# manyeyes/K2TransducerAsr

Measured on AMD Instinct MI355X. Metric: RTFx (audio-sec/wall-sec) offline Zipformer greedy, higher is better.
Workload: dtype f32

## Files before the change

### k2transducerasr_amd/csrc/elementwise.hip

```cpp
#include "kernels.h"

namespace k2hip {
namespace {

constexpr float kLogFloor = -23.025850929940457F;

__device__ __forceinline__ float fast_softplus(float z) { return z > 15.f ? z : __logf(1.0f + __expf(z)); }
__device__ __forceinline__ float swoosh_r(float v) { return fast_softplus(v - 1.0f) - 0.08f * v - 0.313261687f; }
__device__ __forceinline__ float fast_tanh(float v) {
    float e = __expf(-2.0f * fabsf(v));
    float t = (1.0f - e) / (1.0f + e);
    return v < 0.f ? -t : t;
}

__device__ __forceinline__ float sigm(float s) { return 1.0f / (1.0f + __expf(-s)); }
__device__ __forceinline__ float dswish(float v) { return v / (1.0f + __expf(1.0f - v)); }

inline int nblocks(long long n, int per) { return (int)((n + per - 1) / per); }

__global__ void k_pad_logfloor(const float* __restrict__ packed, const long long* __restrict__ off,
                               const long long* __restrict__ len, float* __restrict__ out, long long L) {
    int b = blockIdx.y;
    const float* src = packed + off[b];
    long long n = len[b];
    for (long long j = (long long)blockIdx.x * blockDim.x + threadIdx.x; j < L; j += (long long)gridDim.x * blockDim.x) {
        float v = j < n ? src[j] : 0.0f;
        out[(long long)b * L + j] = (v == 0.0f) ? kLogFloor : v;
    }
}
__global__ void k_pad_logfloor_dense(const float* __restrict__ feats, long long n, float* __restrict__ out, long long L) {
    int b = blockIdx.y;
    for (long long j = (long long)blockIdx.x * blockDim.x + threadIdx.x; j < L; j += (long long)gridDim.x * blockDim.x) {
        float v = j < n ? feats[(long long)b * n + j] : 0.0f;
        out[(long long)b * L + j] = (v == 0.0f) ? kLogFloor : v;
    }
}

template <int TPAD, bool DSWISH>
__global__ void k_conv0(const float* __restrict__ x, const float* __restrict__ w, const float* __restrict__ bias,
                        float* __restrict__ y, int B, int T, int F) {
    __shared__ float sw[72], sb[8];
    if (threadIdx.x < 72) sw[threadIdx.x] = w[threadIdx.x];
    if (threadIdx.x < 8) sb[threadIdx.x] = bias[threadIdx.x];
    __syncthreads();
    int T1 = T - 2 + 2 * TPAD;
    long long n = (long long)B * T1 * F;
    long long i = (long long)blockIdx.x * blockDim.x + threadIdx.x;
    if (i >= n) return;
    int f = (int)(i % F);
    long long bt = i / F;
    int t = (int)(bt % T1), b = (int)(bt / T1);
    float xin[3][3];
#pragma unroll
    for (int kt = 0; kt < 3; kt++)
#pragma unroll
        for (int kf = 0; kf < 3; kf++) {
            int ff = f + kf - 1, tt = t + kt - TPAD;
            xin[kt][kf] = (ff >= 0 && ff < F && tt >= 0 && tt < T) ? x[((long long)b * T + tt) * F + ff] : 0.f;
// ... 719 lines not shown
```

### k2transducerasr_amd/csrc/engine.cpp

```cpp
#include <cstring>
#include <thread>

#include "engine.h"

#include <climits>
#include <cmath>

namespace k2hip {

namespace {
constexpr int kTailFrames = 19;
}

Engine::Engine(const std::string& weights, const char* overrides, int device) : device_(device) {
    tunables_init_from_env();
    model_.reset(new Model(weights, overrides));
    int n = 0;
    if (hipGetDeviceCount(&n) != hipSuccess || n <= 0)
        failf(K2HIP_ERR_NO_DEVICE, "no HIP device visible: libk2hip has no CPU fallback");
    if (device < 0 || device >= n) failf(K2HIP_ERR_NO_DEVICE, "device %d out of range (have %d)", device, n);
    K2_HIP(hipSetDevice(device));
    model_->upload(device);
    K2_HIP(hipStreamCreateWithFlags(&stream_, hipStreamNonBlocking));
    K2_HIP(hipStreamCreateWithFlags(&stream2_, hipStreamNonBlocking));
// ... 1065 lines not shown
    run_sized([&](const Ctx& c) {
        Arena& ar = *c.arena;
        d_tok = ar.take<long long>((int64_t)B * max_tokens);
        d_ts = ar.take<int>((int64_t)B * max_tokens);
        d_n = ar.take<int>(B);
        d_ovf = ar.take<int>(1);
        float* d_packed = ar.take<float>(total);
        long long* d_off = ar.take<long long>(B);
        long long* d_len = ar.take<long long>(B);
        float* d_x = ar.take<float>((int64_t)B * L);
        if (!c.dry) {
            K2_HIP(hipEventRecord(ev_[0], c.stream));
            K2_HIP(hipMemcpyAsync(d_packed, pin, sizeof(float) * total, hipMemcpyHostToDevice, c.stream));
            K2_HIP(hipMemcpyAsync(d_off, off.data(), sizeof(long long) * B, hipMemcpyHostToDevice, c.stream));
            K2_HIP(hipMemcpyAsync(d_len, len.data(), sizeof(long long) * B, hipMemcpyHostToDevice, c.stream));
            K2_HIP(hipEventRecord(ev_[1], c.stream));
        }
        pad_logfloor(c, d_packed, d_off, d_len, d_x, B, L);
        if (!c.dry) K2_HIP(hipEventRecord(ev_[2], c.stream));
        int Tp = 0;
        float* enc = encoder_forward(c, d_x, B, T, &Tp, -1, nullptr, nullptr, nullptr);
        if (!c.dry) K2_HIP(hipEventRecord(ev_[3], c.stream));
        greedy_device(c, enc, B, Tp, single, d_tok, d_ts, d_n, max_tokens, d_ovf);
        if (!c.dry) K2_HIP(hipEventRecord(ev_[4], c.stream));
    });
    finish_tokens(d_tok, d_ts, d_n, d_ovf, B, max_tokens, tokens, ts, n_tokens);
    auto el = [&](int a, int b) { float ms = 0; (void)hipEventElapsedTime(&ms, ev_[a], ev_[b]); return ms; };
    timing_.fbank_ms = 0;
    timing_.pad_ms = el(1, 2);
    timing_.encoder_ms = el(2, 3);
    timing_.greedy_ms = el(3, 4);
    timing_.d2h_ms = el(4, 5);
    timing_.total_ms = el(0, 5);
}

void Engine::offline_greedy_samples_dev(const float* samples_dev, int64_t n_each, int B, int64_t* tokens, int32_t* ts,
                                        int32_t* n_tokens, int max_tokens) {
    K2_REQUIRE(B > 0 && max_tokens > 0 && samples_dev != nullptr, "offline_greedy_from_samples: bad arguments");
    const Config& cf = model_->cfg();
    const FbankOpts& f = cf.fbank;
    K2_REQUIRE(cf.ctc || cf.J == 512, "offline loops hard-code a 512-wide encoder_out; joiner_dim is %d", cf.J);
    const int64_t nf = fbank_num_frames(n_each);
    K2_REQUIRE(nf > 0, "offline_greedy_from_samples: %lld samples give no frame", (long long)n_each);
    const int64_t n_fl = nf * cf.feat, L = n_fl + 80 * kTailFrames;
    const int T = (int)(L / cf.feat);
    long long* d_tok = nullptr;
    int *d_ts = nullptr, *d_n = nullptr, *d_ovf = nullptr;
    run_sized([&](const Ctx& c) {
        Arena& ar = *c.arena;
        d_tok = ar.take<long long>((int64_t)B * max_tokens);
        d_ts = ar.take<int>((int64_t)B * max_tokens);
        d_n = ar.take<int>(B);
        d_ovf = ar.take<int>(1);
        float* d_feats = ar.take<float>((int64_t)B * n_fl);
        float* d_x = ar.take<float>((int64_t)B * L);
        if (!c.dry) K2_HIP(hipEventRecord(ev_[0], c.stream));
        FbankArgs a{samples_dev, n_each, n_each, B, nf, d_feats, model_->d_window, model_->d_melw, f.frame_len, f.frame_shift,
                    f.preemph, f.input_scale, f.remove_dc};
        a.melrange = model_->d_melrange;
        fbank(c, a);
        if (!c.dry) K2_HIP(hipEventRecord(ev_[1], c.stream));
        pad_logfloor_dense(c, d_feats, n_fl, d_x, B, L);
        if (!c.dry) K2_HIP(hipEventRecord(ev_[2], c.stream));
        int Tp = 0;
        float* enc = encoder_forward(c, d_x, B, T, &Tp, -1, nullptr, nullptr, nullptr);
        if (!c.dry) K2_HIP(hipEventRecord(ev_[3], c.stream));
        greedy_device(c, enc, B, Tp, false, d_tok, d_ts, d_n, max_tokens, d_ovf);
        if (!c.dry) K2_HIP(hipEventRecord(ev_[4], c.stream));
    });
    finish_tokens(d_tok, d_ts, d_n, d_ovf, B, max_tokens, tokens, ts, n_tokens);
    auto el = [&](int a, int b) { float ms = 0; (void)hipEventElapsedTime(&ms, ev_[a], ev_[b]); return ms; };
    timing_.fbank_ms = el(0, 1);
    timing_.pad_ms = el(1, 2);
    timing_.encoder_ms = el(2, 3);
    timing_.greedy_ms = el(3, 4);
    timing_.d2h_ms = el(4, 5);
    timing_.total_ms = el(0, 5);
}

void Engine::offline_greedy_samples(const float* const* samples, const int64_t* n_samples, int B, int64_t* tokens, int32_t* ts,
                                    int32_t* n_tokens, int max_tokens, bool single, bool pinned_src) {
    K2_REQUIRE(B > 0 && max_tokens > 0, "offline_greedy_from_samples: bad B=%d / max_tokens=%d", B, max_tokens);
    K2_REQUIRE(!single || B == 1, "offline_greedy_from_samples: the single-stream loop takes one stream");
    K2_HIP(hipSetDevice(device_));
    const Config& cf = model_->cfg();
    const FbankOpts& f = cf.fbank;
    K2_REQUIRE(cf.ctc || cf.J == 512, "offline loops hard-code a 512-wide encoder_out (OfflineRecognizer.cs:103,201); joiner_dim is %d", cf.J);
    int64_t nmax = 0;
    for (int b = 0; b < B; b++) {
        K2_REQUIRE(samples[b] != nullptr && fbank_num_frames(n_samples[b]) > 0, "stream %d: %lld samples give no frame", b, (long long)n_samples[b]);
        nmax = std::max(nmax, n_samples[b]);
    }
    const int64_t nfmax = fbank_num_frames(nmax), n_fl = nfmax * cf.feat, L = n_fl + 80 * kTailFrames;
    const int T = (int)(L / cf.feat);
    const int64_t ns = (nmax + 3) & ~(int64_t)3;
    const int64_t nb_s = align_up((int64_t)sizeof(float) * B * ns, 16);
    const int64_t hb_s = pinned_src ? 0 : nb_s, hb_in = hb_s + 32 * (int64_t)B;
    char* pin = static_cast<char*>(pinned(std::max<int64_t>(hb_in, (int64_t)B * max_tokens * 12 + 4 * (int64_t)B + 64) + 64));
    long long* h_off = reinterpret_cast<long long*>(pin + hb_s);
    long long* h_len = h_off + B;
    const float** h_ptr = reinterpret_cast<const float**>(h_len + B);
    long long* h_cnt = reinterpret_cast<long long*>(h_ptr + B);
    if (pinned_src) {
        for (int b = 0; b < B; b++) {
            void* dp = nullptr;
            K2_HIP(hipHostGetDevicePointer(&dp, const_cast<float*>(samples[b]), 0));
            h_ptr[b] = static_cast<const float*>(dp);
            h_cnt[b] = n_samples[b];
        }
    } else {
        auto stage = [&](int b_lo, int b_hi) {
            for (int b = b_lo; b < b_hi; b++) {
                float* row = reinterpret_cast<float*>(pin) + (size_t)b * ns;
                memcpy(row, samples[b], sizeof(float) * (size_t)n_samples[b]);
                if (n_samples[b] < ns) memset(row + n_samples[b], 0, sizeof(float) * (size_t)(ns - n_samples[b]));
            }
        };
        const int64_t stage_bytes = (int64_t)sizeof(float) * B * ns;
        const int helpers = stage_bytes >= (4 << 20) ? std::min(3, B - 1) : 0;
        if (helpers > 0) {
            std::vector<std::thread> th;
            const int per = (B + helpers) / (helpers + 1);
            for (int h = 1; h <= helpers; h++) th.emplace_back(stage, std::min(B, h * per), std::min(B, (h + 1) * per));
            stage(0, std::min(B, per));
            for (auto& t : th) t.join();
        } else {
            stage(0, B);
        }
    }
    for (int b = 0; b < B; b++) {
        h_off[b] = (long long)b * n_fl;
        h_len[b] = fbank_num_frames(n_samples[b]) * cf.feat;
    }
    long long* d_tok = nullptr;
    int *d_ts = nullptr, *d_n = nullptr, *d_ovf = nullptr;
    run_sized([&](const Ctx& c) {
        Arena& ar = *c.arena;
        d_tok = ar.take<long long>((int64_t)B * max_tokens);
        d_ts = ar.take<int>((int64_t)B * max_tokens);
        d_n = ar.take<int>(B);
        d_ovf = ar.take<int>(1);
        char* d_in = ar.take<char>(nb_s + 32 * (int64_t)B);
        float* d_s = reinterpret_cast<float*>(d_in);
        long long* d_off = reinterpret_cast<long long*>(d_in + nb_s);
        long long* d_len = d_off + B;
        const float* const* d_ptr = reinterpret_cast<const float* const*>(d_len + B);
        const long long* d_cnt = reinterpret_cast<const long long*>(d_ptr + B);
        float* d_feats = ar.take<float>((int64_t)B * n_fl);
        float* d_x = ar.take<float>((int64_t)B * L);
        if (!c.dry) {
            K2_HIP(hipEventRecord(ev_[0], c.stream));
            if (pinned_src) K2_HIP(hipMemcpyAsync(d_in + nb_s, pin, (size_t)(32 * (int64_t)B), hipMemcpyHostToDevice, c.stream));
            else K2_HIP(hipMemcpyAsync(d_in, pin, (size_t)(nb_s + 16 * (int64_t)B), hipMemcpyHostToDevice, c.stream));
        }
        if (pinned_src) gather_samples(c, d_ptr, d_cnt, d_s, B, ns);
        FbankArgs a{d_s, nmax, ns, B, nfmax, d_feats, model_->d_window, model_->d_melw, f.frame_len, f.frame_shift,
                    f.preemph, f.input_scale, f.remove_dc};
        a.melrange = model_->d_melrange;
        fbank(c, a);
        if (!c.dry) K2_HIP(hipEventRecord(ev_[1], c.stream));
        pad_logfloor(c, d_feats, d_off, d_len, d_x, B, L);
        if (!c.dry) K2_HIP(hipEventRecord(ev_[2], c.stream));
        int Tp = 0;
        float* enc = encoder_forward(c, d_x, B, T, &Tp, -1, nullptr, nullptr, nullptr);
        if (!c.dry) K2_HIP(hipEventRecord(ev_[3], c.stream));
        greedy_device(c, enc, B, Tp, single, d_tok, d_ts, d_n, max_tokens, d_ovf);
        if (!c.dry) K2_HIP(hipEventRecord(ev_[4], c.stream));
    });
    finish_tokens(d_tok, d_ts, d_n, d_ovf, B, max_tokens, tokens, ts, n_tokens);
    auto el = [&](int a, int b) { float ms = 0; (void)hipEventElapsedTime(&ms, ev_[a], ev_[b]); return ms; };
    timing_.fbank_ms = el(0, 1);
    timing_.pad_ms = el(1, 2);
    timing_.encoder_ms = el(2, 3);
    timing_.greedy_ms = el(3, 4);
    timing_.d2h_ms = el(4, 5);
    timing_.total_ms = el(0, 5);
}

int Engine::submit_samples_dev(const float* samples_dev, int64_t n_each, int B, int max_tokens) {
    K2_REQUIRE(samples_dev != nullptr, "offline_submit: bad arguments");
    return submit_impl(samples_dev, nullptr, n_each, B, max_tokens);
}
int Engine::submit_samples_host(const float* samples_host, int64_t n_each, int B, int max_tokens) {
    K2_REQUIRE(samples_host != nullptr, "offline_submit: bad arguments");
    return submit_impl(nullptr, samples_host, n_each, B, max_tokens);
}

int Engine::submit_impl(const float* samples_dev, const float* samples_host, int64_t n_each, int B, int max_tokens) {
    K2_REQUIRE(B > 0 && max_tokens > 0, "offline_submit: bad arguments");
    const Config& cf = model_->cfg();
    const FbankOpts& f = cf.fbank;
    K2_REQUIRE(cf.ctc || cf.J == 512, "offline loops hard-code a 512-wide encoder_out; joiner_dim is %d", cf.J);
    const int64_t nf = fbank_num_frames(n_each);
    K2_REQUIRE(nf > 0, "offline_submit: %lld samples give no frame", (long long)n_each);
    const bool deep = beam_ > 0 && !cf.ctc;
    const int nslots = deep ? kSlots : 2;
    int ticket = -1, in_flight = 0;
    for (const auto& x : slots_) in_flight += x.busy;
    for (int k = 0; k < kSlots && ticket < 0; k++) {
        const int cand = (next_slot_ + k) % kSlots;
        if (!slots_[cand].busy && cand < nslots) ticket = cand;
    }
    if (ticket < 0 || in_flight >= nslots)
        failf(K2HIP_ERR_INVALID, "offline_submit: %d batches already in flight; wait for one first", in_flight);
    Slot& sl = slots_[ticket];
    if (!sl.stream) K2_HIP(hipStreamCreateWithFlags(&sl.stream, hipStreamNonBlocking));
    const int64_t n_fl = nf * cf.feat, L = n_fl + 80 * kTailFrames;
    const int T = (int)(L / cf.feat);
    const int64_t nb = (int64_t)B * max_tokens * 12 + (int64_t)B * 4 + 64;
    if (nb > sl.pin_cap) {
        if (sl.pin) K2_HIP(hipHostFree(sl.pin));
        sl.pin = nullptr;
        sl.pin_cap = 0;
        K2_HIP(hipHostMalloc(&sl.pin, (size_t)nb, hipHostMallocDefault));
        sl.pin_cap = nb;
    }
    cur_arena_ = &sl.arena;
    hipStream_t s2 = deep ? sl.stream : stream2_;
    try {
        run_sized([&](const Ctx& c) {
            Arena& ar = *c.arena;
            sl.d_tok = ar.take<long long>((int64_t)B * max_tokens);
            sl.d_ts = ar.take<int>((int64_t)B * max_tokens);
            sl.d_n = ar.take<int>(B);
            sl.d_ovf = ar.take<int>(1);
            float* d_feats = ar.take<float>((int64_t)B * n_fl);
            float* d_x = ar.take<float>((int64_t)B * L);
            const float* src = samples_dev;
            if (samples_host) {
                float* d_s = ar.take<float>((int64_t)B * n_each);
                src = d_s;
                if (!c.dry) {
                    hipStream_t cs = deep ? stream2_ : sl.stream;
                    K2_HIP(hipMemcpyAsync(d_s, samples_host, sizeof(float) * (size_t)B * n_each, hipMemcpyHostToDevice, cs));
                    K2_HIP(hipEventRecord(sl.h2d_done, cs));
                    K2_HIP(hipStreamWaitEvent(c.stream, sl.h2d_done, 0));
                }
            }
            FbankArgs a{src, n_each, n_each, B, nf, d_feats, model_->d_window, model_->d_melw, f.frame_len, f.frame_shift,
                        f.preemph, f.input_scale, f.remove_dc};
            a.melrange = model_->d_melrange;
            fbank(c, a);
            pad_logfloor_dense(c, d_feats, n_fl, d_x, B, L);
            int Tp = 0;
            float* enc = encoder_forward(c, d_x, B, T, &Tp, -1, nullptr, nullptr, nullptr);
            Ctx cd = c;
            cd.stream = s2;
            cd.instrument = false;
            cd.greedy_rec = &sl.greedy;
            sl.greedy.valid = false;
            if (!c.dry) {
                K2_HIP(hipEventRecord(sl.enc_done, c.stream));
                K2_HIP(hipStreamWaitEvent(s2, sl.enc_done, 0));
            }
            greedy_device(cd, enc, B, Tp, false, sl.d_tok, sl.d_ts, sl.d_n, max_tokens, sl.d_ovf);
        });
    } catch (...) {
        cur_arena_ = &arena_;
        throw;
    }
    cur_arena_ = &arena_;
    const int64_t nb_tok = (int64_t)B * max_tokens * 8, nb_ts = (int64_t)B * max_tokens * 4, nb_n = (int64_t)B * 4;
    char* pin = static_cast<char*>(sl.pin);
    K2_HIP(hipMemcpyAsync(pin, sl.d_tok, nb_tok, hipMemcpyDeviceToHost, s2));
    K2_HIP(hipMemcpyAsync(pin + nb_tok, sl.d_ts, nb_ts, hipMemcpyDeviceToHost, s2));
    K2_HIP(hipMemcpyAsync(pin + nb_tok + nb_ts, sl.d_n, nb_n, hipMemcpyDeviceToHost, s2));
    K2_HIP(hipMemcpyAsync(pin + nb_tok + nb_ts + nb_n, sl.d_ovf, 4, hipMemcpyDeviceToHost, s2));
    K2_HIP(hipEventRecord(sl.done, s2));
    sl.B = B;
    sl.max_tokens = max_tokens;
    sl.search_stream = s2;
    sl.busy = true;
    next_slot_ = (ticket + 1) % nslots;
    return ticket;
}

void Engine::wait_ticket(int ticket, int64_t* tokens, int32_t* ts, int32_t* n_tokens) {
    K2_REQUIRE(ticket >= 0 && ticket < kSlots && slots_[ticket].busy, "offline_wait: ticket %d is not in flight", ticket);
    K2_HIP(hipSetDevice(device_));
    Slot& sl = slots_[ticket];
    K2_HIP(hipEventSynchronize(sl.done));
    sl.busy = false;
    const int64_t nb_tok = (int64_t)sl.B * sl.max_tokens * 8, nb_ts = (int64_t)sl.B * sl.max_tokens * 4, nb_n = (int64_t)sl.B * 4;
    char* pin = static_cast<char*>(sl.pin);
    int ovf = *reinterpret_cast<const int*>(pin + nb_tok + nb_ts + nb_n);
    note_search(sl.greedy.valid && sl.greedy.a.overflow == sl.d_ovf, ovf == 2 && sl.greedy.valid && sl.greedy.a.overflow == sl.d_ovf);
    if (ovf == 2 && sl.greedy.valid && sl.greedy.a.overflow == sl.d_ovf) {
        hipStream_t s2 = sl.search_stream;
        greedy_relaunch_one_part(s2, sl.greedy);
        search_retries_++;
        K2_HIP(hipMemcpyAsync(pin, sl.d_tok, nb_tok, hipMemcpyDeviceToHost, s2));
        K2_HIP(hipMemcpyAsync(pin + nb_tok, sl.d_ts, nb_ts, hipMemcpyDeviceToHost, s2));
        K2_HIP(hipMemcpyAsync(pin + nb_tok + nb_ts, sl.d_n, nb_n, hipMemcpyDeviceToHost, s2));
        K2_HIP(hipMemcpyAsync(pin + nb_tok + nb_ts + nb_n, sl.d_ovf, 4, hipMemcpyDeviceToHost, s2));
        K2_HIP(hipStreamSynchronize(s2));
        ovf = *reinterpret_cast<const int*>(pin + nb_tok + nb_ts + nb_n);
// ... 421 lines not shown
        } else if (name == "lstm_cell") {
            float* gx = P();
            const long long ldgx = L();
            float* gh = P();
            const int ldgh = I();
            float *cc = P(), *hf = P();
            const int B = I(), Hh = I();
            lstm_cell(c, gx, ldgx, gh, ldgh, cc, hf, B, Hh);
        } else if (name == "lstm_cell_rows") {
            float *gates = P(), *cc = P(), *hf = P();
            const int rows = I(), Hh = I();
            lstm_cell_rows(c, gates, cc, hf, rows, Hh);
        } else if (name == "lstm_add_frame") {
            float* Y = P();
            const long long SY = L();
            float* hp = P();
            const long long pstride = L();
            const int S = I();
            float *h = P(), *x1 = P();
            const int n = I(), B = I(), T = I(), D = I(), lo = I(), s = I();
            lstm_add_frame(c, Y, SY, hp, pstride, S, h, x1, n, B, T, D, lo, s);
        } else if (name == "lstm_norm_frame") {
            float *x1 = P(), *fp = P();
            const long long pstride = L();
            const int S = I();
            float *b2 = P(), *eps = P();
            const long long lstride = L();
            float* Y = P();
            const long long SY = L();
            const int n = I(), B = I(), T = I(), D = I(), lo = I(), s = I();
            lstm_norm_frame(c, x1, fp, pstride, S, b2, eps, lstride, Y, SY, n, B, T, D, lo, s);
        } else if (name == "add_inplace") {
            float *a = P(), *b = P();
            const long long n = L();
            add_inplace(c, a, b, n);
        } else if (name == "gather_rows" || name == "scatter_rows") {
            float* pool = P();
            const long long ss = L(), off = L();
            const int* slots = reinterpret_cast<const int*>(P());
            float* io = P();
            if (name == "gather_rows") {
                const int B = I(), width = I();
                gather_rows(c, pool, ss, off, slots, io, B, width);
            } else {
                const int ldin = I(), B = I(), width = I();
                scatter_rows(c, pool, ss, off, slots, io, ldin, B, width);
            }
        } else if (name == "greedy_screen_counts") {
            float* out = P();
            K2_REQUIRE(out && buf_bytes[0] >= 16, "debug_op_run greedy_screen_counts: a buffer of 2 int64 is needed");
            K2_HIP(hipStreamSynchronize(stream_));
            K2_HIP(copy_blocking(out, d_screen_counts_, 2 * sizeof(unsigned long long), hipMemcpyDeviceToDevice));
            out_mask |= 1u;
        } else if (name == "basicnorm") {
            float *x = P(), *le = P(), *y = P();
            const int M = I(), D = I();
            basicnorm(c, x, le, y, M, D);
        } else if (name == "conv0_pad1_dswish" || name == "conv0_nopad_dswish") {
            float *x = P(), *w = P(), *b = P(), *y = P();
            const int B = I(), T = I(), Fq = I();
            if (name == "conv0_pad1_dswish") conv0_pad1_dswish(c, x, w, b, y, B, T, Fq);
            else conv0_nopad_dswish(c, x, w, b, y, B, T, Fq);
        } else {
            failf(K2HIP_ERR_INVALID, "debug_op_run: unknown op '%s'", op);
        }
    } catch (const Error& e) {
        if (e.code == K2HIP_ERR_INVALID && strncmp(e.what(), "debug_op_run", 12) != 0) throw Error(K2HIP_ERR_UNSUPPORTED, e.what());
        throw;
    }
    if (!took) failf(K2HIP_ERR_UNSUPPORTED, "debug_op_run %s: the launcher does not take this shape", op);
    K2_REQUIRE(ni == n_iargs && nbuf == n_bufs, "debug_op_run %s: %d int arguments and %d buffers passed, %d and %d used", op, n_iargs, n_bufs, ni,
               nbuf);
    K2_HIP(hipStreamSynchronize(stream_));
    std::vector<unsigned char> g((size_t)kGuard);
    for (int k = 0; k < n_bufs; k++) {
        if (!dev[k]) continue;
        const char* p = static_cast<const char*>(dev[k]);
        for (int side = 0; side < 2; side++) {
            K2_HIP(copy_blocking(g.data(), side ? p + buf_bytes[k] : p - kGuard, (size_t)kGuard, hipMemcpyDeviceToHost));
            for (int64_t i = 0; i < kGuard; i++)
                if (g[(size_t)i] != 0xff)
                    failf(K2HIP_ERR_INVALID, "debug_op_run %s: buffer %d written %s its end (guard byte %lld)", op, k, side ? "past" : "before",
                          (long long)(side ? i : kGuard - i));
        }
    }
    for (int k = 0; k < n_bufs; k++)
        if (dev[k] && (out_mask >> k & 1u)) K2_HIP(copy_blocking(bufs[k], dev[k], (size_t)buf_bytes[k], hipMemcpyDeviceToHost));
}

void Engine::debug_gemm_trace(int M, int N, int K, int act, bool with_res, int cfg, unsigned long long* out, int64_t cap, int* n_wg, int* n_waves) {
    K2_HIP(hipSetDevice(device_));
    GemmForceGuard force(cfg);
    GemmArgs g;
    g.lda = K; g.ldw = K; g.ldc = N; g.M = M; g.N = N; g.K = K; g.act = act; g.ldr = N;
    const GemmPlan p = plan_gemm(g, gemm_force());
    K2_REQUIRE(p.family == GemmFamily::DMA || p.family == GemmFamily::RING || p.family == GemmFamily::PIPE,
               "trace: LDS-DMA (0, 5, 7, 9, 10, 11), ring (100+) and pipelined (2000+) configurations only");
    *n_wg = cdiv(M, p.BM) * cdiv(N, p.BN);
    *n_waves = p.waves;
    const int64_t words = (int64_t)*n_wg * p.waves * 64;
    K2_REQUIRE(words <= cap, "trace buffer too small: need %lld words", (long long)words);
    std::vector<float> h((size_t)std::max((int64_t)M * K, std::max((int64_t)N * K, (int64_t)M * N)));
    uint32_t s = 12345u;
    for (auto& v : h) { s = s * 1664525u + 1013904223u; v = ((s >> 8) * (1.0f / 8388608.0f)) - 1.0f; }
    DevBufs dev;
    float* A = dev.alloc<float>((size_t)M * K);
// ... 54 lines not shown
```

### k2transducerasr_amd/csrc/fbank.hip

```cpp
#include <cfloat>
#include <mutex>
#include <vector>

#include "kernels.h"

namespace k2hip {
namespace {

constexpr int NFFT = 512, NBIN = 256, LOG2N = 9;

__global__ __launch_bounds__(256) void k_fbank(FbankArgs a, const double2* __restrict__ tw, int num_mel) {
    __shared__ double re[NFFT], im[NFFT];
    __shared__ double red[4];
    const int tid = threadIdx.x, lane = tid & 63, wave = tid >> 6;
    const long long f = blockIdx.x;
    const int u = blockIdx.y;
    const float* s = a.samples + (long long)u * a.utt_stride + f * a.frame_shift;
    const int N = a.frame_len;

    double x0 = 0.0, x1 = 0.0, p0 = 0.0, p1 = 0.0;
    const double scale = (double)a.input_scale;
    int i0 = tid, i1 = tid + 256;
    if (i0 < N) { x0 = (double)s[i0] * scale; p0 = (double)s[i0 > 0 ? i0 - 1 : 0] * scale; }
    if (i1 < N) { x1 = (double)s[i1] * scale; p1 = (double)s[i1 - 1] * scale; }
    if (a.remove_dc) {
        double part = x0 + x1;
#pragma unroll
        for (int o = 32; o > 0; o >>= 1) part += __shfl_xor(part, o);
        if (lane == 0) red[wave] = part;
        __syncthreads();
        double mean = (red[0] + red[1] + red[2] + red[3]) / (double)N;
        x0 -= mean; x1 -= mean; p0 -= mean; p1 -= mean;
    }
    if (a.preemph != 0.f) {
        x0 = x0 - (double)a.preemph * p0;
        x1 = x1 - (double)a.preemph * p1;
    }
    if (i0 < N) x0 *= (double)a.window[i0]; else x0 = 0.0;
    if (i1 < N) x1 *= (double)a.window[i1]; else x1 = 0.0;
    re[__brev((unsigned)i0) >> (32 - LOG2N)] = x0;
    re[__brev((unsigned)i1) >> (32 - LOG2N)] = x1;
    im[i0] = 0.0;
    im[i1] = 0.0;
    __syncthreads();
#pragma unroll
    for (int st = 0; st < LOG2N; st++) {
        int hl = 1 << st;
        int k = tid & (hl - 1);
        int i = ((tid >> st) << (st + 1)) + k;
        int j = i + hl;
        double2 w = tw[k << (LOG2N - 1 - st)];
        double xr = re[j] * w.x - im[j] * w.y, xi = re[j] * w.y + im[j] * w.x;
        double ar = re[i], ai = im[i];
        re[j] = ar - xr; im[j] = ai - xi;
        re[i] = ar + xr; im[i] = ai + xi;
        __syncthreads();
    }
    double pw = re[tid] * re[tid] + im[tid] * im[tid];
    __syncthreads();
    re[tid] = pw;
    __syncthreads();
    float* out = a.feats + ((long long)u * a.n_frames + f) * num_mel;
    if (tid < num_mel) {
        const int lo = (int)a.melrange[2 * tid], hi = (int)a.melrange[2 * tid + 1];
        const float* w = a.melw + tid * NBIN;
        double e = 0.0;
        for (int k = lo; k < hi; k++) e += (double)w[k] * re[k];
        float ef = (float)e;
        if (ef < FLT_EPSILON) ef = FLT_EPSILON;
        out[tid] = logf(ef);
    }
}

std::mutex g_tw_mu;
double2* g_tw[16] = {nullptr};

const double2* twiddles(int device) {
    if (device < 0 || device >= 16) failf(K2HIP_ERR_INVALID, "device index %d out of range", device);
    std::lock_guard<std::mutex> lk(g_tw_mu);
    if (!g_tw[device]) {
        std::vector<double2> h(NBIN);
        for (int k = 0; k < NBIN; k++) {
            double ang = -2.0 * M_PI * k / NFFT;
            h[k].x = cos(ang);
            h[k].y = sin(ang);
        }
        double2* d = nullptr;
        K2_HIP(hipMalloc(&d, sizeof(double2) * NBIN));
        if (hipError_t e = copy_blocking(d, h.data(), sizeof(double2) * NBIN, hipMemcpyHostToDevice); e != hipSuccess) {
            (void)hipFree(d);
            K2_HIP(e);
        }
        g_tw[device] = d;
    }
    return g_tw[device];
}

}

void fbank(const Ctx& ctx, const FbankArgs& a) {
    if (a.n_frames <= 0 || a.n_utts <= 0) return;
    K2_REQUIRE(a.frame_len <= NFFT && a.frame_len > 256, "fbank: frame_len %d unsupported", a.frame_len);
    K2_REQUIRE(a.melrange != nullptr, "fbank: mel filter extents missing");
    if (ctx.dry) return;
    int dev = 0;
    K2_HIP(hipGetDevice(&dev));
    const double2* tw = twiddles(dev);
    dim3 grid((unsigned)a.n_frames, (unsigned)a.n_utts);
    hipLaunchKernelGGL(k_fbank, grid, dim3(256), 0, ctx.stream, a, tw, 80);
    K2_HIP(hipGetLastError());
}

__global__ __launch_bounds__(256) void k_gather_samples(const float* const* __restrict__ src, const long long* __restrict__ n,
                                                        float* __restrict__ dst, long long nmax) {
    const int b = blockIdx.y;
    const float* s = src[b];
    const long long cnt = n[b];
    float* d = dst + (long long)b * nmax;
    const bool al = ((reinterpret_cast<unsigned long long>(s) | reinterpret_cast<unsigned long long>(d)) & 15) == 0;
    for (long long i4 = (long long)blockIdx.x * 256 + threadIdx.x; 4 * i4 < nmax; i4 += (long long)gridDim.x * 256) {
        const long long i = 4 * i4;
        if (al && i + 3 < cnt && i + 3 < nmax) {
            *reinterpret_cast<float4*>(d + i) = *reinterpret_cast<const float4*>(s + i);
        } else {
            for (int k = 0; k < 4 && i + k < nmax; k++) d[i + k] = i + k < cnt ? s[i + k] : 0.f;
        }
    }
}

void gather_samples(const Ctx& ctx, const float* const* src, const long long* n, float* dst, int B, long long nmax) {
    if (ctx.dry) return;
    K2_REQUIRE(B > 0 && nmax > 0, "gather_samples: empty batch");
    const int gx = (int)std::min<long long>(cdiv((int)std::min<long long>((nmax + 3) / 4, 1 << 30), 256), 64);
    hipLaunchKernelGGL(k_gather_samples, dim3(gx, B), dim3(256), 0, ctx.stream, src, n, dst, nmax);
    K2_HIP(hipGetLastError());
}

}
```

### k2transducerasr_amd/csrc/kernels.h

```cpp
#pragma once
#include "common.h"

namespace k2hip {

#ifdef K2HIP_DEV
#define K2HIP_DEV_SWITCH(name, def) int name = def
#else
#define K2HIP_DEV_SWITCH(name, def) static constexpr int name = def
#endif
struct Tunables {
    int no_glu_epilogue = 0;
    int attn_long = 0;
    int no_fused_av = 0;
    int fused_vproj_min_t = 4;
    int no_fused_vproj = 0;
    int no_fused_conv = 0;
    int conformer_gemm_scores = 0;
    int dw7_tiled = 0;
    int dw1d_tt = 0;
    int lstm_seq = 0;
    int greedy_one_part = 0;
    int greedy_parts = 0;
    int beam_launches = 0;
    int beam_parts = 0;
// ... 123 lines not shown
    X(5, 128, 64, 32, 32, 32) X(12, 128, 32, 32, 32, 32)
enum GemmMode { MODE_PLAIN = 0, MODE_CONV = 1, MODE_WKN = 2 };

enum class GemmFamily { REG, DMA, PIPE, P16, RING, SKINNY3, SKINNY6, SKINNY6_8 };
struct GemmPlan {
    GemmFamily family = GemmFamily::REG;
    int idx = 0;
    int mode = MODE_PLAIN;
    int ablate = 0;
    int BM = 0, BN = 0, waves = 0;
};
struct GemmForce {
    enum Kind { AUTO, CFG, RING, PIPE, P16 } kind = AUTO;
    int idx = -1;
    int ablate = 0;
    bool dma = true;
};
GemmForce decode_gemm_force(int code);
GemmPlan plan_gemm(const GemmArgs& a, const GemmForce& f);
int gemm_kind(const GemmArgs& a, const GemmPlan& p);
int glu_conv_ring_entry(int B, int Tc, int D, int K);
void debug_force_gemm_cfg(int code);
GemmForce gemm_force();
struct GemmForceGuard {
    explicit GemmForceGuard(int code) { debug_force_gemm_cfg(code); }
    ~GemmForceGuard() { debug_force_gemm_cfg(-1); }
    GemmForceGuard(const GemmForceGuard&) = delete;
    GemmForceGuard& operator=(const GemmForceGuard&) = delete;
};
void linear(const Ctx& ctx, const float* A, int lda, const float* W, const float* bias, float* C, int ldc, int M, int K,
            int N, int act = ACT_NONE, const float* res = nullptr, int ldr = 0);

struct RingRef {
    float* pool = nullptr;
    long long slot_stride = 0;
    long long off = 0;
    const int* slots = nullptr;
    const int* chunks = nullptr;
};

void attn_scores_softmax(const Ctx& ctx, const float* qkp, int ld, const float* pp, float* aw, int B, int T, int Tp, int H, int qh = 32,
                         int koff0 = -1, int poff0 = -1);

bool attn_av_out(const Ctx& ctx, const float* aw, const float* v, const float* wout, const float* bias, float* x, int B, int T, int KL, int Tp,
                 int H, int vh, int D);
bool attn_av_out_ring(const Ctx& ctx, const float* aw, const RingRef& vals, const float* newrows, const float* wout, const float* bias, float* x,
                      int B, int T, int KL, int Tp, int H, int vh, int D);
void attn_proj_av_out_ring(const Ctx& ctx, const float* aw, const RingRef& vals, const float* xin, const float* win, const float* bin,
                           const float* wout, const float* bias, float* xout, int B, int T, int KL, int Tp, int H, int vh, int D);

void nonlin_av_out_ring(const Ctx& ctx, const float* aw, const RingRef& cache, const float* hid, int ldh, const float* wout, const float* bias,
                        float* x, int B, int T, int KL, int Tp, int Hc, int D);

void pad_logfloor(const Ctx& ctx, const float* packed, const long long* d_off, const long long* d_len, float* out, int B,
                  long long L);
void pad_logfloor_dense(const Ctx& ctx, const float* feats, long long n_each, float* out, int B, long long L);
void conv0_swoosh(const Ctx& ctx, const float* x, const float* w, const float* b, float* y, int B, int T, int F);
void conv0_pad1_dswish(const Ctx& ctx, const float* x, const float* w, const float* b, float* y, int B, int T, int F);
void dwconv7x7(const Ctx& ctx, const float* x, const float* w_kc, const float* b, float* y, int B, int Tin, int Tout, int tpad,
               int F, int C);
void biasnorm(const Ctx& ctx, const float* x, const float* bias, const float* log_scale, float* y, int M, int D);
void biasnorm_bypass(const Ctx& ctx, const float* x, const float* orig, const float* nbias, const float* log_scale,
                     const float* scale, float* y, int M, int D);
void biasnorm_bypass_downsample(const Ctx& ctx, const float* x, const float* orig, const float* nbias, const float* log_scale, const float* scale,
                                float* y, const float* bias2, float* xd2, int B, int T, int D, int ds2, int D2);
struct LayerTail {
    const float* bias2 = nullptr;
    float* xd2 = nullptr;
    int ds2 = 1, D2 = 0;
};
void bypass(const Ctx& ctx, const float* orig, const float* x, const float* scale, float* y, int M, int D);
void glu_sigmoid(const Ctx& ctx, const float* x, float* y, int M, int D);
void tanh_gate(const Ctx& ctx, const float* x, float* y, int M, int Hc);
void mul_cols(const Ctx& ctx, float* a, const float* x, int ldx, int col0, int M, int N);
void dwconv1d_swoosh(const Ctx& ctx, const float* x, const float* w_kd, const float* b, float* y, int B, int T, int D, int K);
void glu_dwconv1d_swoosh(const Ctx& ctx, const float* x2, const float* w_kd, const float* b, float* y, int B, int T, int D,
                          int K);
void glu_dwconv1d_dswish(const Ctx& ctx, const float* x2, const float* w_kd, const float* b, float* y, int B, int T, int D,
                          int K);
void conv0_nopad_dswish(const Ctx& ctx, const float* x, const float* w, const float* b, float* y, int B, int T, int F);
void lstm_cell(const Ctx& ctx, const float* gx, long long ldgx, const float* gh, int ldgh, float* c, float* hf, int B, int Hh);
void add_inplace(const Ctx& ctx, float* a, const float* b, long long n);
void lstm_cell_rows(const Ctx& ctx, const float* gates, float* c, float* hf, int rows, int Hh);
void lstm_add_frame(const Ctx& ctx, const float* Y, long long SY, const float* hp, long long pstride, int S, float* h, float* x1, int n, int B,
                    int T, int D, int lo, int s);
void lstm_norm_frame(const Ctx& ctx, const float* x1, const float* fp, long long pstride, int S, const float* b2_0, const float* eps0,
                     long long lstride, float* Y, long long SY, int n, int B, int T, int D, int lo, int s);
void gather_rows(const Ctx& ctx, const float* pool, long long slot_stride, long long off, const int* slots, float* out, int B, int width);
void scatter_rows(const Ctx& ctx, float* pool, long long slot_stride, long long off, const int* slots, const float* in, int ldin, int B, int width);
void basicnorm(const Ctx& ctx, const float* x, const float* log_eps, float* y, int M, int D);
void conformer_qprep(const Ctx& ctx, const float* qkv, const float* bias_u, const float* bias_v, float* qu, float* qv, int M,
                     int D, float scaling, int ldq = 0 );
void conformer_softmax_shift_stream(const Ctx& ctx, float* ac, const float* bd, const long long* plen, int B, int H, int Tc, int left,
                                    int KLp, int NPp);
void slice_rows(const Ctx& ctx, const float* in, float* out, int B, int Tin, int row0, int Tout, int D);
void dwconv_valid_dswish(const Ctx& ctx, const float* cat, const float* w_kd, const float* bias, float* y, int B, int Tc, int D, int K);
void conformer_softmax_shift(const Ctx& ctx, float* ac, const float* bd, int Z, int T, int Tp, int NPp);
bool conformer_scores_softmax(const Ctx& ctx, const float* qu, const float* qv, const float* kmat, int ldk, const float* pp, float* aw, int B, int H,
                              int T, int Tp, int D, int ldq = 0, const float* bias_u = nullptr, const float* bias_v = nullptr, float scaling = 1.0f);
void downsample(const Ctx& ctx, const float* x, const float* bias, float* y, int B, int T, int D, int ds, int Din = 0);
void upsample_combine(const Ctx& ctx, const float* orig, const float* xd, const float* scale, float* y, int B, int T,
                      int Td, int D, int ds, int Dorig = 0);
void upsample_combine_downsample(const Ctx& ctx, const float* orig, const float* xd, const float* scale, float* y, const float* bias2,
                                 float* xd2, int B, int T, int Td, int D, int ds, int Dorig, int D2, int ds2);
void convert_channels(const Ctx& ctx, const float* x, float* y, int M, int Din, int Dout);
struct FullDimSegs {
    const float* src[8];
    int ld[8], col1[8], n = 0;
    const float* lz_orig = nullptr;
    const float* lz_xd = nullptr;
    const float* lz_scale = nullptr;
    int lz_Td = 0, lz_ds = 1, lz_Do = 0;
};
void downsample_full(const Ctx& ctx, const FullDimSegs& segs, const float* bias, float* y, int B, int T, int D, int ds);
void copy_cols(const Ctx& ctx, const float* x, int ldx, int xcol0, float* y, int ldy, int ycol0, int M, int n);

struct FbankArgs {
    const float* samples;
    long long n_samples;
    long long utt_stride;
    int n_utts;
    long long n_frames;
    float* feats;
    const float* window;
    const float* melw;
    int frame_len, frame_shift;
    float preemph, input_scale;
    int remove_dc;
    const float* melrange = nullptr;
};
void fbank(const Ctx& ctx, const FbankArgs& a);
void gather_samples(const Ctx& ctx, const float* const* src, const long long* n, float* dst, int B, long long nmax);

struct DecJoinW {
    const float* emb;
    const float* conv;
    int cpg;
    const float* ptab = nullptr;
    const float* dproj_kn;
    const float* dproj_b;
    const float* out_kn;
    const float* out_b;
    const float* dec_table = nullptr;
    const void* out_h16 = nullptr;
    const float* out_eps = nullptr;
    const float* out_vj = nullptr;
    int V, Vp, DD, J, ctx;
};
void decoder(const Ctx& ctx, const DecJoinW& w, const long long* y, int N, float* dec_out);
void decoder_start_contexts(const Ctx& ctx, const DecJoinW& w, float* out);
void decoder_table(const Ctx& ctx, const DecJoinW& w, float* table);
void decoder_rows_wide(const Ctx& ctx, const DecJoinW& w, const long long* y, int N, float* out);
void tanh_add(const Ctx& ctx, const float* enc, const float* dec, int dec_stride, float* y, int N, int J);
void argmax_rows(const Ctx& ctx, const float* logits, int ld, int N, int V, int* tok);
void log_softmax_rows(const Ctx& ctx, float* x, int M, int V);
void argmax_first_rows(const Ctx& ctx, const float* logits, int ld, int N, int V, int* tok);
void ctc_collapse(const Ctx& ctx, const int* tok, int B, int Tp, const int* frame_off, long long* tokens, int* timestamps,
                  int* n_tokens, int max_tokens, int* trail, int* any, int* overflow);
void first_emit_frame(const Ctx& ctx, const int* tok, int B, int Tp, int skip1, int* t0);
struct GreedyArgs {
    const float* enc;
    int B, Tp;
    const int* t0;
    int skip1;
    int max_sym;
    long long* tokens;
    int* timestamps;
    int* n_tokens;
    int max_tokens;
    int* overflow;
    const long long* init_ctx = nullptr;
    int parts = 1;
    unsigned long long* gran = nullptr;
    unsigned long long* gran2 = nullptr;
    const float* dec_init = nullptr;
    unsigned long long* stamps = nullptr;
    unsigned long long* screen_counts = nullptr;
};
void greedy_loop(const Ctx& ctx, const DecJoinW& w, const GreedyArgs& a);
bool greedy_loop_screens(const DecJoinW& w, int B, bool streaming, bool one_part);
struct BeamHwStream {
    const int* next = nullptr;
    const float* bonus = nullptr;
    const float* pending = nullptr;
// ... 164 lines not shown
```

Before: 23730.

## Fuse log-floor padding into a multi-frame radix-8 fbank kernel

Replaces the per-frame radix-2 FFT fbank kernel with one where each block handles a span of up to 16 frames. Each wave runs a register-resident radix-8 FFT, samples are staged once in shared memory, and the mel projection is done from a transposed power table. The kernel writes straight into the padded encoder input with the log-floor fill, which removes the separate pad_logfloor pass and the intermediate feature buffer. The old kernel stays reachable as fbank_radix2 for testing. It also adds fma contraction choices and frame-length checks, and takes on more complex shared-memory use and bounds logic.

Result: no change. 23900 (median of 6 runs) (+0.7%).

```diff
diff --git a/k2transducerasr_amd/csrc/elementwise.hip b/k2transducerasr_amd/csrc/elementwise.hip
--- a/k2transducerasr_amd/csrc/elementwise.hip
+++ b/k2transducerasr_amd/csrc/elementwise.hip
@@ -2,8 +2,6 @@
 
 namespace k2hip {
 namespace {
-
-constexpr float kLogFloor = -23.025850929940457F;
 
 __device__ __forceinline__ float fast_softplus(float z) { return z > 15.f ? z : __logf(1.0f + __expf(z)); }
 __device__ __forceinline__ float swoosh_r(float v) { return fast_softplus(v - 1.0f) - 0.08f * v - 0.313261687f; }
diff --git a/k2transducerasr_amd/csrc/engine.cpp b/k2transducerasr_amd/csrc/engine.cpp
--- a/k2transducerasr_amd/csrc/engine.cpp
+++ b/k2transducerasr_amd/csrc/engine.cpp
@@ -1141,15 +1141,14 @@
         d_ts = ar.take<int>((int64_t)B * max_tokens);
         d_n = ar.take<int>(B);
         d_ovf = ar.take<int>(1);
-        float* d_feats = ar.take<float>((int64_t)B * n_fl);
         float* d_x = ar.take<float>((int64_t)B * L);
         if (!c.dry) K2_HIP(hipEventRecord(ev_[0], c.stream));
-        FbankArgs a{samples_dev, n_each, n_each, B, nf, d_feats, model_->d_window, model_->d_melw, f.frame_len, f.frame_shift,
+        FbankArgs a{samples_dev, n_each, n_each, B, nf, d_x, model_->d_window, model_->d_melw, f.frame_len, f.frame_shift,
                     f.preemph, f.input_scale, f.remove_dc};
         a.melrange = model_->d_melrange;
+        a.out_stride = a.out_len = L;
         fbank(c, a);
         if (!c.dry) K2_HIP(hipEventRecord(ev_[1], c.stream));
-        pad_logfloor_dense(c, d_feats, n_fl, d_x, B, L);
         if (!c.dry) K2_HIP(hipEventRecord(ev_[2], c.stream));
         int Tp = 0;
         float* enc = encoder_forward(c, d_x, B, T, &Tp, -1, nullptr, nullptr, nullptr);
@@ -1187,8 +1186,8 @@
     const int64_t hb_s = pinned_src ? 0 : nb_s, hb_in = hb_s + 32 * (int64_t)B;
     char* pin = static_cast<char*>(pinned(std::max<int64_t>(hb_in, (int64_t)B * max_tokens * 12 + 4 * (int64_t)B + 64) + 64));
     long long* h_off = reinterpret_cast<long long*>(pin + hb_s);
-    long long* h_len = h_off + B;
-    const float** h_ptr = reinterpret_cast<const float**>(h_len + B);
+    long long* h_nfr = h_off + B;
+    const float** h_ptr = reinterpret_cast<const float**>(h_nfr + B);
     long long* h_cnt = reinterpret_cast<long long*>(h_ptr + B);
     if (pinned_src) {
         for (int b = 0; b < B; b++) {
@@ -1218,8 +1217,8 @@
         }
     }
     for (int b = 0; b < B; b++) {
-        h_off[b] = (long long)b * n_fl;
-        h_len[b] = fbank_num_frames(n_samples[b]) * cf.feat;
+        h_off[b] = 0;
+        h_nfr[b] = fbank_num_frames(n_samples[b]);
     }
     long long* d_tok = nullptr;
     int *d_ts = nullptr, *d_n = nullptr, *d_ovf = nullptr;
@@ -1232,10 +1231,9 @@
         char* d_in = ar.take<char>(nb_s + 32 * (int64_t)B);
         float* d_s = reinterpret_cast<float*>(d_in);
         long long* d_off = reinterpret_cast<long long*>(d_in + nb_s);
-        long long* d_len = d_off + B;
-        const float* const* d_ptr = reinterpret_cast<const float* const*>(d_len + B);
+        const long long* d_nfr = d_off + B;
+        const float* const* d_ptr = reinterpret_cast<const float* const*>(d_nfr + B);
         const long long* d_cnt = reinterpret_cast<const long long*>(d_ptr + B);
-        float* d_feats = ar.take<float>((int64_t)B * n_fl);
         float* d_x = ar.take<float>((int64_t)B * L);
         if (!c.dry) {
             K2_HIP(hipEventRecord(ev_[0], c.stream));
@@ -1243,12 +1241,13 @@
             else K2_HIP(hipMemcpyAsync(d_in, pin, (size_t)(nb_s + 16 * (int64_t)B), hipMemcpyHostToDevice, c.stream));
         }
         if (pinned_src) gather_samples(c, d_ptr, d_cnt, d_s, B, ns);
-        FbankArgs a{d_s, nmax, ns, B, nfmax, d_feats, model_->d_window, model_->d_melw, f.frame_len, f.frame_shift,
+        FbankArgs a{d_s, nmax, ns, B, nfmax, d_x, model_->d_window, model_->d_melw, f.frame_len, f.frame_shift,
                     f.preemph, f.input_scale, f.remove_dc};
         a.melrange = model_->d_melrange;
+        a.out_stride = a.out_len = L;
+        a.out_frames = d_nfr;
         fbank(c, a);
         if (!c.dry) K2_HIP(hipEventRecord(ev_[1], c.stream));
-        pad_logfloor(c, d_feats, d_off, d_len, d_x, B, L);
         if (!c.dry) K2_HIP(hipEventRecord(ev_[2], c.stream));
         int Tp = 0;
         float* enc = encoder_forward(c, d_x, B, T, &Tp, -1, nullptr, nullptr, nullptr);
@@ -1313,7 +1312,6 @@
             sl.d_ts = ar.take<int>((int64_t)B * max_tokens);
             sl.d_n = ar.take<int>(B);
             sl.d_ovf = ar.take<int>(1);
-            float* d_feats = ar.take<float>((int64_t)B * n_fl);
             float* d_x = ar.take<float>((int64_t)B * L);
             const float* src = samples_dev;
             if (samples_host) {
@@ -1326,11 +1324,11 @@
                     K2_HIP(hipStreamWaitEvent(c.stream, sl.h2d_done, 0));
                 }
             }
-            FbankArgs a{src, n_each, n_each, B, nf, d_feats, model_->d_window, model_->d_melw, f.frame_len, f.frame_shift,
+            FbankArgs a{src, n_each, n_each, B, nf, d_x, model_->d_window, model_->d_melw, f.frame_len, f.frame_shift,
                         f.preemph, f.input_scale, f.remove_dc};
             a.melrange = model_->d_melrange;
+            a.out_stride = a.out_len = L;
             fbank(c, a);
-            pad_logfloor_dense(c, d_feats, n_fl, d_x, B, L);
             int Tp = 0;
             float* enc = encoder_forward(c, d_x, B, T, &Tp, -1, nullptr, nullptr, nullptr);
             Ctx cd = c;
@@ -1858,6 +1856,31 @@
             K2_HIP(hipStreamSynchronize(stream_));
             K2_HIP(copy_blocking(out, d_screen_counts_, 2 * sizeof(unsigned long long), hipMemcpyDeviceToDevice));
             out_mask |= 1u;
+        } else if (name == "fbank" || name == "fbank_radix2") {
+            FbankArgs a{};
+            a.samples = P();
+            a.n_samples = L(); a.utt_stride = L(); a.n_utts = I(); a.n_frames = L();
+            a.feats = P(); a.window = P(); a.melw = P();
+            a.frame_len = I(); a.frame_shift = I(); a.preemph = F(); a.input_scale = F(); a.remove_dc = I();
+            a.melrange = P();
+            a.out_stride = L(); a.out_len = L();
+            a.out_frames = reinterpret_cast<const long long*>(P());
+            if (name == "fbank") fbank(c, a);
+            else fbank_radix2(c, a);
+        } else if (name == "pad_logfloor_dense") {
+            float *feats = P(), *out = P();
+            const long long n_each = L();
+            const int B = I();
+            const long long Lr = L();
+            pad_logfloor_dense(c, feats, n_each, out, B, Lr);
+        } else if (name == "pad_logfloor") {
+            float* packed = P();
+            const long long* off = reinterpret_cast<const long long*>(P());
+            const long long* len = reinterpret_cast<const long long*>(P());
+            float* out = P();
+            const int B = I();
+            const long long Lr = L();
+            pad_logfloor(c, packed, off, len, out, B, Lr);
         } else if (name == "basicnorm") {
             float *x = P(), *le = P(), *y = P();
             const int M = I(), D = I();
diff --git a/k2transducerasr_amd/csrc/fbank.hip b/k2transducerasr_amd/csrc/fbank.hip
--- a/k2transducerasr_amd/csrc/fbank.hip
+++ b/k2transducerasr_amd/csrc/fbank.hip
@@ -1,15 +1,197 @@
 #include <cfloat>
+#include <cstdint>
 #include <mutex>
 #include <vector>
 
 #include "kernels.h"
 
+#pragma clang fp contract(off)
+
 namespace k2hip {
 namespace {
 
-constexpr int NFFT = 512, NBIN = 256, LOG2N = 9;
-
-__global__ __launch_bounds__(256) void k_fbank(FbankArgs a, const double2* __restrict__ tw, int num_mel) {
+constexpr int NFFT = 512, NBIN = 256, LOG2N = 9, NMEL = 80;
+constexpr int SPAN = 16;
+constexpr int STAGE_CAP = 2912;
+constexpr int FFT_LD = NFFT + NFFT / 8;
+constexpr int PW_LD = SPAN + 1;
+
+__device__ __forceinline__ void bfly(double& ar, double& ai, double& br, double& bi, const double2 w) {
+    const double xr = fma(br, w.x, -(bi * w.y)), xi = fma(br, w.y, bi * w.x);
+    br = ar - xr; bi = ai - xi;
+    ar = ar + xr; ai = ai + xi;
+}
+
+template <int P>
+__device__ __forceinline__ void radix8(double (&re)[8], double (&im)[8], int low, const double2* tw) {
+    constexpr int S = 1 << (3 * P);
+#pragma unroll
+    for (int s = 0; s < 3; s++) {
+        const int h = 1 << s;
+#pragma unroll
+        for (int m = 0; m < 8; m++) {
+            if (m & h) continue;
+            const int k = (m & (h - 1)) * S + low;
+            bfly(re[m], im[m], re[m + h], im[m + h], tw[k << (LOG2N - 1 - 3 * P - s)]);
+        }
+    }
+}
+
+__device__ __forceinline__ void wave_sync() {
+    __builtin_amdgcn_fence(__ATOMIC_RELEASE, "workgroup");
+    __builtin_amdgcn_wave_barrier();
+    __builtin_amdgcn_fence(__ATOMIC_ACQUIRE, "workgroup");
+}
+
+__global__ __launch_bounds__(256) void k_fbank_span(FbankArgs a, const double2* __restrict__ twg, int span) {
+    __shared__ double2 fft[4][FFT_LD];
+    __shared__ double2 tw[NBIN];
+    __shared__ float smp[STAGE_CAP];
+    static_assert(sizeof(double) * NBIN * PW_LD <= sizeof(double2) * 4 * FFT_LD, "power spectra do not fit the FFT regions");
+    static_assert(SPAN * NMEL <= STAGE_CAP, "features do not fit the sample stage");
+    const int tid = threadIdx.x, lane = tid & 63, wave = tid >> 6;
+    const int u = blockIdx.y;
+    const long long f0 = (long long)blockIdx.x * span;
+    const int N = a.frame_len, shift = a.frame_shift;
+    const bool padded = a.out_len > 0;
+    const int nout = (int)min((long long)span, a.n_frames - f0);
+    long long own = a.n_frames;
+    if (padded && a.out_frames) own = min(own, a.out_frames[u]);
+    const int nfr = (int)max(0LL, min((long long)span, own - f0));
+
+    tw[tid] = twg[tid];
+    if (nfr > 0) {
+        const float* src = a.samples + (long long)u * a.utt_stride + f0 * shift;
+        const int cnt = (nfr - 1) * shift + N;
+        const int mis = (int)((reinterpret_cast<uintptr_t>(src) >> 2) & 3);
+        for (int i = 4 * tid - mis; i < cnt; i += 4 * 256) {
+            if (i >= 0 && i + 3 < cnt) {
+                const float4 q = *reinterpret_cast<const float4*>(src + i);
+                smp[i] = q.x; smp[i + 1] = q.y; smp[i + 2] = q.z; smp[i + 3] = q.w;
+            } else {
+#pragma unroll
+                for (int e = 0; e < 4; e++)
+                    if (i + e >= 0 && i + e < cnt) smp[i + e] = src[i + e];
+            }
+        }
+    }
+    const int i_lane = (int)(__brev((unsigned)lane) >> 26);
+    double win[8];
+#pragma unroll
+    for (int m = 0; m < 8; m++) {
+        const int i = (int)(__brev((unsigned)m) >> 29) * 64 + i_lane;
+        win[m] = i < N ? (double)a.window[i] : 0.0;
+    }
+    __syncthreads();
+
+    const double scale = (double)a.input_scale;
+    double2* F = fft[wave];
+    double pw[4][4];
+#pragma unroll
+    for (int q = 0; q < 4; q++) {
+#pragma unroll
+        for (int m = 0; m < 4; m++) pw[q][m] = 0.0;
+        const int fr = wave + 4 * q;
+        if (fr >= nfr) continue;
+        const float* s = smp + fr * shift;
+        double mean = 0.0;
+        if (a.remove_dc) {
+            double red[4];
+#pragma unroll
+            for (int w4 = 0; w4 < 4; w4++) {
+                const int i0 = w4 * 64 + lane, i1 = i0 + 256;
+                const double x0 = (double)s[i0] * scale, x1 = i1 < N ? (double)s[i1] * scale : 0.0;
+                double part = x0 + x1;
+#pragma unroll
+                for (int o = 32; o > 0; o >>= 1) part += __shfl_xor(part, o);
+                red[w4] = part;
+            }
+            mean = (red[0] + red[1] + red[2] + red[3]) / (double)N;
+        }
+        double re[8], im[8];
+#pragma unroll
+        for (int m = 0; m < 8; m++) {
+            const int i = (int)(__brev((unsigned)m) >> 29) * 64 + i_lane;
+            double x = 0.0;
+            if (i < N) {
+                x = (double)s[i] * scale;
+                double p = (double)s[i > 0 ? i - 1 : 0] * scale;
+                if (a.remove_dc) { x -= mean; p -= mean; }
+                if (a.preemph != 0.f) x = fma(-p, (double)a.preemph, x);
+                x *= win[m];
+            }
+            re[m] = x;
+            im[m] = 0.0;
+        }
+        radix8<0>(re, im, 0, tw);
+#pragma unroll
+        for (int m = 0; m < 8; m++) F[9 * lane + m] = make_double2(re[m], im[m]);
+        wave_sync();
+        const int e1 = (lane >> 3) * 72 + (lane & 7);
+#pragma unroll
+        for (int m = 0; m < 8; m++) {
+            const double2 v = F[e1 + 9 * m];
+            re[m] = v.x; im[m] = v.y;
+        }
+        radix8<1>(re, im, lane & 7, tw);
+#pragma unroll
+        for (int m = 0; m < 8; m++) F[e1 + 9 * m] = make_double2(re[m], im[m]);
+        wave_sync();
+        const int e2 = lane + (lane >> 3);
+#pragma unroll
+        for (int m = 0; m < 8; m++) {
+            const double2 v = F[e2 + 72 * m];
+            re[m] = v.x; im[m] = v.y;
+        }
+        radix8<2>(re, im, lane, tw);
+        wave_sync();
+#pragma unroll
+        for (int m = 0; m < 4; m++) pw[q][m] = fma(re[m], re[m], im[m] * im[m]);
+    }
+    __syncthreads();
+    double* P = reinterpret_cast<double*>(&fft[0][0]);
+#pragma unroll
+    for (int q = 0; q < 4; q++)
+#pragma unroll
+        for (int m = 0; m < 4; m++) P[(lane + 64 * m) * PW_LD + wave + 4 * q] = pw[q][m];
+    __syncthreads();
+    float* ft = smp;
+    for (int c = tid; c < NMEL * SPAN; c += 256) {
+        const int fl = c / SPAN, fr = c % SPAN;
+        if (fr >= nfr) continue;
+        const int lo = max((int)a.melrange[2 * fl], 0), hi = min((int)a.melrange[2 * fl + 1], NBIN);
+        const float* w = a.melw + fl * NBIN;
+        double e = 0.0;
+        for (int k = lo; k < hi; k += 4) {
+            const int k1 = min(k + 1, hi - 1), k2 = min(k + 2, hi - 1), k3 = min(k + 3, hi - 1);
+            const double w0 = (double)w[k], w1 = (double)w[k1], w2 = (double)w[k2], w3 = (double)w[k3];
+            const double p0 = P[k * PW_LD + fr], p1 = P[k1 * PW_LD + fr], p2 = P[k2 * PW_LD + fr], p3 = P[k3 * PW_LD + fr];
+            e = fma(w0, p0, e);
+            if (k + 1 < hi) e = fma(w1, p1, e);
+            if (k + 2 < hi) e = fma(w2, p2, e);
+            if (k + 3 < hi) e = fma(w3, p3, e);
+        }
+        float ef = (float)e;
+        if (ef < FLT_EPSILON) ef = FLT_EPSILON;
+        ft[fr * NMEL + fl] = logf(ef);
+    }
+    __syncthreads();
+    if (!padded) {
+        float* dst = a.feats + ((long long)u * a.n_frames + f0) * NMEL;
+        for (int i = tid; i < nfr * NMEL; i += 256) dst[i] = ft[i];
+        return;
+    }
+    float* row = a.feats + (long long)u * a.out_stride;
+    float* dst = row + f0 * NMEL;
+    for (int i = tid; i < nout * NMEL; i += 256) {
+        const float v = i < nfr * NMEL ? ft[i] : 0.0f;
+        dst[i] = v == 0.0f ? kLogFloor : v;
+    }
+    if (blockIdx.x == gridDim.x - 1)
+        for (long long j = a.n_frames * NMEL + tid; j < a.out_len; j += 256) row[j] = kLogFloor;
+}
+
+__global__ __launch_bounds__(256) void k_fbank_radix2(FbankArgs a, const double2* __restrict__ tw, int num_mel) {
     __shared__ double re[NFFT], im[NFFT];
     __shared__ double red[4];
     const int tid = threadIdx.x, lane = tid & 63, wave = tid >> 6;
@@ -33,8 +215,8 @@
         x0 -= mean; x1 -= mean; p0 -= mean; p1 -= mean;
     }
     if (a.preemph != 0.f) {
-        x0 = x0 - (double)a.preemph * p0;
-        x1 = x1 - (double)a.preemph * p1;
+        x0 = fma(-p0, (double)a.preemph, x0);
+        x1 = fma(-p1, (double)a.preemph, x1);
     }
     if (i0 < N) x0 *= (double)a.window[i0]; else x0 = 0.0;
     if (i1 < N) x1 *= (double)a.window[i1]; else x1 = 0.0;
@@ -49,14 +231,13 @@
         int k = tid & (hl - 1);
         int i = ((tid >> st) << (st + 1)) + k;
         int j = i + hl;
-        double2 w = tw[k << (LOG2N - 1 - st)];
-        double xr = re[j] * w.x - im[j] * w.y, xi = re[j] * w.y + im[j] * w.x;
-        double ar = re[i], ai = im[i];
-        re[j] = ar - xr; im[j] = ai - xi;
-        re[i] = ar + xr; im[i] = ai + xi;
+        double ar = re[i], ai = im[i], br = re[j], bi = im[j];
+        bfly(ar, ai, br, bi, tw[k << (LOG2N - 1 - st)]);
+        re[j] = br; im[j] = bi;
+        re[i] = ar; im[i] = ai;
         __syncthreads();
     }
-    double pw = re[tid] * re[tid] + im[tid] * im[tid];
+    double pw = fma(re[tid], re[tid], im[tid] * im[tid]);
     __syncthreads();
     re[tid] = pw;
     __syncthreads();
@@ -65,7 +246,7 @@
         const int lo = (int)a.melrange[2 * tid], hi = (int)a.melrange[2 * tid + 1];
         const float* w = a.melw + tid * NBIN;
         double e = 0.0;
-        for (int k = lo; k < hi; k++) e += (double)w[k] * re[k];
+        for (int k = lo; k < hi; k++) e = fma((double)w[k], re[k], e);
         float ef = (float)e;
         if (ef < FLT_EPSILON) ef = FLT_EPSILON;
         out[tid] = logf(ef);
@@ -100,14 +281,34 @@
 
 void fbank(const Ctx& ctx, const FbankArgs& a) {
     if (a.n_frames <= 0 || a.n_utts <= 0) return;
+    K2_REQUIRE(a.frame_len <= NFFT && a.frame_len > 256 && a.frame_shift > 0, "fbank: frame_len %d / frame_shift %d unsupported", a.frame_len,
+               a.frame_shift);
+    K2_REQUIRE(a.melrange != nullptr, "fbank: mel filter extents missing");
+    if (a.out_len > 0)
+        K2_REQUIRE(a.out_len >= a.n_frames * NMEL && a.out_stride >= a.out_len, "fbank: padded rows of %lld floats (stride %lld) for %lld frames",
+                   a.out_len, a.out_stride, a.n_frames);
+    else
+        K2_REQUIRE(a.out_frames == nullptr && a.out_stride == 0, "fbank: per-utterance frame counts need the padded form");
+    if (ctx.dry) return;
+    int dev = 0;
+    K2_HIP(hipGetDevice(&dev));
+    const double2* tw = twiddles(dev);
+    const int span = std::min(SPAN, 1 + (STAGE_CAP - a.frame_len) / a.frame_shift);
+    dim3 grid((unsigned)cdiv(a.n_frames, (long long)span), (unsigned)a.n_utts);
+    hipLaunchKernelGGL(k_fbank_span, grid, dim3(256), 0, ctx.stream, a, tw, span);
+    K2_HIP(hipGetLastError());
+}
+
+void fbank_radix2(const Ctx& ctx, const FbankArgs& a) {
+    if (a.n_frames <= 0 || a.n_utts <= 0) return;
     K2_REQUIRE(a.frame_len <= NFFT && a.frame_len > 256, "fbank: frame_len %d unsupported", a.frame_len);
-    K2_REQUIRE(a.melrange != nullptr, "fbank: mel filter extents missing");
+    K2_REQUIRE(a.melrange != nullptr && a.out_len == 0, "fbank_radix2: mel filter extents missing, or the padded form asked for");
     if (ctx.dry) return;
     int dev = 0;
     K2_HIP(hipGetDevice(&dev));
     const double2* tw = twiddles(dev);
     dim3 grid((unsigned)a.n_frames, (unsigned)a.n_utts);
-    hipLaunchKernelGGL(k_fbank, grid, dim3(256), 0, ctx.stream, a, tw, 80);
+    hipLaunchKernelGGL(k_fbank_radix2, grid, dim3(256), 0, ctx.stream, a, tw, NMEL);
     K2_HIP(hipGetLastError());
 }
 
diff --git a/k2transducerasr_amd/csrc/kernels.h b/k2transducerasr_amd/csrc/kernels.h
--- a/k2transducerasr_amd/csrc/kernels.h
+++ b/k2transducerasr_amd/csrc/kernels.h
@@ -199,6 +199,7 @@
 void nonlin_av_out_ring(const Ctx& ctx, const float* aw, const RingRef& cache, const float* hid, int ldh, const float* wout, const float* bias,
                         float* x, int B, int T, int KL, int Tp, int Hc, int D);
 
+constexpr float kLogFloor = -23.025850929940457F;
 void pad_logfloor(const Ctx& ctx, const float* packed, const long long* d_off, const long long* d_len, float* out, int B,
                   long long L);
 void pad_logfloor_dense(const Ctx& ctx, const float* feats, long long n_each, float* out, int B, long long L);
@@ -275,8 +276,11 @@
     float preemph, input_scale;
     int remove_dc;
     const float* melrange = nullptr;
+    long long out_stride = 0, out_len = 0;
+    const long long* out_frames = nullptr;
 };
 void fbank(const Ctx& ctx, const FbankArgs& a);
+void fbank_radix2(const Ctx& ctx, const FbankArgs& a);
 void gather_samples(const Ctx& ctx, const float* const* src, const long long* n, float* dst, int B, long long nmax);
 
 struct DecJoinW {
```
